# OpenGene/repaq

Hardware: AMD Instinct MI355X
Metric: raw FASTQ MB/s encode+decode (higher is better)
Workload: dtype u8; 1 GPU; configs[2]: synthetic NovaSeq PE150 two files (-i/-I), 2 x 4.01 GB FASTQ (fqgen profile 1, 11200000 pairs, seed 3, N 20 ppm), -k 1000, encode + decode; chunks_per_gpu=3360, parity=unchecked (checked with --full)

## Files before the change

repaq_amd/csrc/enc/gather_tiles.h:

```cpp
#pragma once
#define G2_CAP 23552u
#define G2_SE_OK 1
#define G2_CNT 256u
__device__ __forceinline__ uint32_t ctl_flags4(uint32_t w) { return (w - 0x10101010u) & ~w & 0x80808080u; }
struct __attribute__((packed, aligned(1))) GU16g { uint32_t a, b, c, d; };
__device__ __forceinline__ void pack4_codes(uint32_t w, uint32_t& code, uint32_t& nb, uint32_t& bad) {
    const uint32_t idx = (w >> 1) & 0x03030303u;
    const uint32_t ok = eq_bytes_full(__builtin_amdgcn_perm(0u, 0x47544341u, idx), w);
    code = ((__builtin_amdgcn_perm(0u, 0x00020301u, idx) & ok) * 0x01041040u) >> 24;
    nb = 0; bad = 0;
    if (ok != 0xFFFFFFFFu) { const uint32_t isn = eq_bytes_full(w, 0x4E4E4E4Eu); nb = ((isn & 0x01010101u) * 0x01020408u) >> 24;
            bad = (((~ok & ~isn) & 0x01010101u) * 0x01020408u) >> 24; }
}
__device__ __forceinline__ void pack4_codes_rc(uint32_t w, uint32_t& code, uint32_t& nb) {
    const uint32_t u = w & 0xDFDFDFDFu, idx = (u >> 1) & 0x03030303u;
    const uint32_t ok = eq_bytes_full(__builtin_amdgcn_perm(0u, 0x47544341u, idx), u);
    code = ((__builtin_amdgcn_perm(0u, 0x03010002u, idx) & ok) * 0x01041040u) >> 24;
    nb = ((~ok & 0x01010101u) * 0x01020408u) >> 24;
}
__device__ __forceinline__ bool pack16_fast(const uint32_t (&w)[4], uint32_t& code) {
    uint32_t diff = 0; code = 0;
#pragma unroll
    for (int i = 0; i < 4; i++) {
        const uint32_t idx = (w[i] >> 1) & 0x03030303u;
// ... 461 lines not shown
    G2MRaw mr = g2_mraw(T, pq, gs, j, ntile ? tile_at(1) - gs : 0u);
    if (ntile) g2_stage<SH>(T, two, g2_geo<SH>(b0, b1, two), buf4, tid);
    for (uint32_t t = 0; t < ntile; t++, tix++) {
        const uint32_t cur = tile_at(t), cnt = tile_at(t + 1u) - cur;
        const G2Geo g = g2_geo<SH>(b0, b1, two);
        const G2Read m = g2_read(T, mr, g, f, pq0, il, cur, j, cnt);
        const uint32_t qbeg = b0.q - pq0, qend = b1.q - pq0;
        { const uint32_t ncur = tile_at(t + 1u); mr = g2_mraw(T, pq, ncur, j, tile_at(t + 2u) - ncur); }
        const G2Bound b3 = g2_bound<SH>(T, two, pq, tile_at(t + 3u));
        __syncthreads();
        if (LANES) { if (m.on && (m.gi & 1u)) { const uint32_t ts = m.ssrc + m.len + 1u;
                if (g2_ctl_line(tx, m.nsrc, m.ssrc - 1u - m.nsrc, part, P) | g2_ctl_line(tx, ts, m.qsrc - 1u - ts, part, P)) s_mctl = 1u; } }
        qc.seg0 = qbeg / PC_SEG_POS;
        if (parse && (uint32_t)wave_id() == (tix & 3u)) { g2_parse(T, R, tx, REFN, REFS, g, r0, f, cur, cnt, can0, dpos, dch, acc);
                if (mirror || LANES) g2_mirror_ends(T, tx, g, cur, cnt, M.mirror_err, LANES); }
        if (MASKS) {
            if (tid < nd && s_carry[tid]) atomicOr(&pl[tid * M.pw], s_carry[tid]);
            g2_quals_masks<LANES>(tx, m, part, P, pl, M.pw, qbeg & ~31u, nd, pat0, pat1, pat2, patm, D, qd, gpl, M.pstride, segm + (size_t)c * MAX_STREAMS * n_seg,
                    segc + (size_t)c * MAX_STREAMS * n_seg, n_seg, M.rare + (size_t)c * (1u + G2_RARE_LIST), &s_mctl);
            g2_bases<LANES>(tx, m, part, P, lpk, lnb, rflag, rn, &s_mctl);
        } else g2_compose(tx, m, part, P, qd, lpk, lnb, rflag, rn, qc);
        if (mirror) {
            const uint32_t end1 = g.end1 < T.n[1] ? g.end1 : T.n[1];
            const uint32_t mctl = wave_sum(g2_ctl_count(buf4 + g.base1 / 16u, b0.l1 - g.a01, end1 - g.a01, tid));
            if ((tid & 63u) == 0 && mctl) atomicAdd(&s_mctl, mctl);
            mwant += 2u * cnt - (g.end1 > T.n[1] ? 1u : 0u);
        }
        __syncthreads();
        if (t + 1u < ntile) g2_stage<SH>(T, two, g2_geo<SH>(b1, b2, two), buf4, tid);
        if (MASKS) {
            const uint32_t gw0 = qbeg >> 5, nw = ((qend + 31u) >> 5) - gw0; const bool last_tile = cur + cnt >= ge;
            g2_flush_masks(pl, M.pw, nd, dense3, s_carry, gpl, M.pstride, gw0, nw, !last_tile && (qend & 31u) != 0u, cur == gs && gs > f && (qbeg & 31u) != 0u,
                    last_tile && ge < e && (qend & 31u) != 0u,
                           (size_t)c * MAX_STREAMS * n_seg, n_seg, segm, segc);
        } else qual_flush(sh, sh_last, nrep, nslot, qc.seg0, c, nn_s, segm, segc, n_seg);
        b0 = b1; b1 = b2; b2 = b3;
    }
    if (parse) {
        const uint32_t bits = wave_and(acc.bits), fail = wave_min(acc.fail);
        if ((tid & 63u) == 0) { if (bits != CF_ALL) atomicAnd(&cbits[c], bits); if (fail != 0xFFFFFFFFu) atomicMin(&cfail[c], fail); }
    }
    if (mirror) {
        __syncthreads();
        if (tid == 0 && s_mctl != mwant) atomicOr(M.mirror_err, (uint32_t)DE_MIRROR_FAIL);
    }
    if (LANES) { __syncthreads(); if (tid == 0 && s_mctl) atomicOr(M.mirror_err, (uint32_t)DE_MIRROR_FAIL); }
}
__device__ __forceinline__ uint32_t dense_mask_of(const DevHeader* __restrict__ D, uint32_t nd) { uint32_t m = 0;
        for (uint32_t d = 0; d < nd; d++) m |= 1u << D->dense[d]; return m; }
__device__ __forceinline__ void k_rare_zero_chunk(uint32_t* __restrict__ planes, uint64_t pstride, uint32_t dense_mask, const uint32_t* __restrict__ pq,
        const uint32_t* __restrict__ first, const uint64_t* __restrict__ qbase, uint32_t c) {
    const uint32_t nw = (pq[first[c + 1]] - pq[first[c]] + 31u) >> 5; const size_t w0 = (size_t)(qbase[c] >> 5);
    for (uint32_t v = 0; v < G2_PLANES; v++) if (!((dense_mask >> v) & 1u)) for (uint32_t i = threadIdx.x; i < nw; i += blockDim.x) planes[(size_t)v * pstride + w0 + i] = 0u;
}
__device__ __forceinline__ void nbits_zero_slots(uint16_t* __restrict__ lnb, const uint8_t* __restrict__ rn, const uint32_t* __restrict__ pq, uint32_t g0, uint32_t g1, uint32_t t, uint32_t n) {
    for (uint32_t g = g0 + t; g < g1; g += n) if (rn[g]) { const uint32_t a = pq[g], nw = (pq[g + 1] - a + 15u) >> 4; uint16_t* const o = lnb + (size_t)(a >> 4) + g;
            for (uint32_t i = 0; i < nw; i++) o[i] = 0; }
}
__global__ void k_gather_redo_reset(const uint32_t* __restrict__ only, uint32_t* __restrict__ segm, int* __restrict__ segc, uint32_t n_seg,
                                    uint32_t* __restrict__ xplane, uint64_t pstride, const DevHeader* __restrict__ D, uint32_t nd, const uint32_t* __restrict__ pq, const uint32_t* __restrict__ first, const uint64_t* __restrict__ qbase,
                                    uint16_t* __restrict__ lnb, const uint8_t* __restrict__ rn) {
    const uint32_t c = blockIdx.x; if (!only[c]) return;
    nbits_zero_slots(lnb, rn, pq, first[c], first[c + 1], threadIdx.x, blockDim.x);
    const size_t k = (size_t)c * MAX_STREAMS * n_seg;
    for (uint32_t i = threadIdx.x; i < MAX_STREAMS * n_seg; i += blockDim.x) { segm[k + i] = 0u; segc[k + i] = -1; }
    if (xplane) { k_rare_zero_chunk(xplane, pstride, dense_mask_of(D, nd), pq, first, qbase, c);
            if (threadIdx.x == 0) xplane[(size_t)G2_PLANES * pstride + (size_t)c * (1u + G2_RARE_LIST)] = 0u; }
}
__global__ void k_rare_cleanup(uint32_t* __restrict__ rare, uint32_t* __restrict__ planes, uint64_t pstride, const DevHeader* __restrict__ D, uint32_t nd,
        const uint32_t* __restrict__ pq, const uint32_t* __restrict__ first, const uint64_t* __restrict__ qbase) {
    const uint32_t c = blockIdx.x; uint32_t* const rc = rare + (size_t)c * (1u + G2_RARE_LIST); const uint32_t n = rc[0]; if (!n) return;
    if (n <= G2_RARE_LIST) { const size_t w0 = (size_t)(qbase[c] >> 5); for (uint32_t i = threadIdx.x; i < n; i += blockDim.x) { const uint32_t e = rc[1u + i];
            planes[(size_t)(e >> 28) * pstride + w0 + (e & 0x0FFFFFFFu)] = 0u; } }
    else k_rare_zero_chunk(planes, pstride, dense_mask_of(D, nd), pq, first, qbase, c);
    __syncthreads();
    if (threadIdx.x == 0) rc[0] = 0u;
}
__global__ void __launch_bounds__(256) k_nbits_cleanup(uint16_t* __restrict__ lnb, const uint8_t* __restrict__ rn, const uint32_t* __restrict__ pq, uint32_t n_reads) {
    const uint32_t g0 = 16u * (blockIdx.x * blockDim.x + threadIdx.x); if (g0 >= n_reads) return;
    const uint4 v = *(const uint4*)(rn + g0);
    if (!(v.x | v.y | v.z | v.w)) return;
    nbits_zero_slots(lnb, rn, pq, g0, g0 + 16u < n_reads ? g0 + 16u : n_reads, 0u, 1u);
}
__device__ __forceinline__ uint32_t loose_codes(const uint32_t* __restrict__ lpk, uint32_t ld, uint32_t b) {
    const uint32_t d = ld + (b >> 4), sh = 2u * (b & 15u); const uint32_t lo = lpk[d];
    return sh ? (uint32_t)(((((unsigned long long)lpk[d + 1]) << 32) | lo) >> sh) : lo;
}
__device__ __forceinline__ uint32_t loose_nbits(const uint16_t* __restrict__ lnb, uint32_t ld, uint32_t b) {
    const uint32_t d = ld + (b >> 4), sh = b & 15u; const uint32_t lo = lnb[d];
    return (sh ? ((((uint32_t)lnb[d + 1]) << 16) | lo) >> sh : lo) & 0xFFFFu;
}
#define SP_OWN 4096u
#define SP_EXTRA 8u
#define SP_U 3
struct __attribute__((packed, aligned(4))) SpU8 { uint32_t a, b; };
struct __attribute__((packed, aligned(2))) SpU4 { uint32_t a; };
__global__ void __launch_bounds__(256) k_seqpack(const uint32_t* __restrict__ pq, const uint32_t* __restrict__ sd, const U4* __restrict__ ptot,
        const uint32_t* __restrict__ first, const uint32_t* __restrict__ ilv, const int8_t* __restrict__ ovb,
                                                 const DevHeader* __restrict__ D, const uint64_t* __restrict__ sbase, const uint32_t* __restrict__ lpk, const uint16_t* __restrict__ lnb, const uint8_t* __restrict__ rn,
                                                 uint32_t* __restrict__ spk, uint16_t* __restrict__ snm, uint32_t* __restrict__ ncount, uint32_t* __restrict__ nmap, uint32_t* __restrict__ segm, int* __restrict__ segc, uint32_t n_seg,
                                                 uint32_t rshift) {
    __shared__ uint32_t s_sd[256 + SP_EXTRA + 1], s_ld[256 + SP_EXTRA], s_sk[256 + SP_EXTRA]; __shared__ uint8_t s_own[SP_OWN];
    __shared__ uint8_t s_hn[256 + SP_EXTRA + 8];
    const uint32_t c = blockIdx.y, f = first[c], e = first[c + 1], tid = threadIdx.x;
    const uint32_t ps0 = sd[f], S = ptot[c].d;
    const bool il = ilv[c] != 0, enc = il && (D->flags & H_PE_OVERLAP); const int shift = D->overlap_shift;
    uint32_t* const ok = spk + (size_t)(sbase[c] >> 4); uint16_t* const on = snm + (size_t)(sbase[c] >> 4);
    const uint32_t nshift = nmap_shift(S); uint32_t* const nm = nmap + (size_t)c * NMAP_WORDS;
    const size_t nsi = ((size_t)c * MAX_STREAMS + NPOS_SLOT) * n_seg;
    uint32_t nsum = 0;
    auto skip_of = [&](uint32_t g) -> uint32_t {
        if (enc && ((g - f) & 1u)) { const int ov = (int)ovb[g >> 1] - shift; if (ov > 0) return (uint32_t)ov; }
        return 0u;
    };
    const uint32_t R = 1u << rshift;
    for (uint32_t r0 = f + blockIdx.x * R; r0 < e; r0 += gridDim.x * R) {
        const uint32_t nr = e - r0 < R ? e - r0 : R, nx = e - r0 < R + SP_EXTRA ? e - r0 : R + SP_EXTRA;
        for (uint32_t t = tid; t <= nx; t += blockDim.x) {
            const uint32_t g = r0 + t; s_sd[t] = g < e ? sd[g] - ps0 : S;
            if (t < nx) { s_ld[t] = (pq[g] >> 4) + g; s_sk[t] = skip_of(g); s_hn[t] = rn[g]; } else s_hn[t] = 0;
        }
        __syncthreads();
        const uint32_t kbase = (s_sd[0] + 15u) >> 4, kend = (s_sd[nr] + 15u) >> 4;
        if (tid < nr) { const uint32_t ka = (s_sd[tid] + 15u) >> 4, kb = (s_sd[tid + 1] + 15u) >> 4; for (uint32_t k = ka; k < kb; k++) s_own[k - kbase] = (uint8_t)tid; }
        __syncthreads();
        const uint32_t ndw = kend - kbase;
        for (uint32_t i0 = 0; i0 < ndw; i0 += blockDim.x * SP_U) {
            struct Dw { uint32_t k, need, t1, jj, sh, sh2, take2, n, n2; unsigned long long c, c2; } q[SP_U]; uint32_t nres[SP_U];
#pragma unroll
            for (int u = 0; u < SP_U; u++) nres[u] = 0;
#pragma unroll
            for (int u = 0; u < SP_U; u++) {
                Dw& x = q[u]; x.need = 0; x.take2 = 0; x.k = x.t1 = x.jj = x.sh = x.sh2 = x.n = x.n2 = 0; x.c = x.c2 = 0;
                const uint32_t i = i0 + (uint32_t)u * blockDim.x + tid;
                if (i < ndw) {
                    const uint32_t k = kbase + i, j = s_own[i];
                    const uint32_t B = 16u * k, si = B - s_sd[j], need = S - B < 16u ? S - B : 16u, av = s_sd[j + 1] - B, t1 = need < av ? need : av;
                    const uint32_t b0 = s_sk[j] + si, d = s_ld[j] + (b0 >> 4);
                    x.k = k; x.need = need; x.t1 = t1; x.sh = b0 & 15u; x.jj = j + 1u;
                    { const SpU8 v = *(const SpU8*)(lpk + d); x.c = (((unsigned long long)v.b) << 32) | v.a; x.n = s_hn[j] ? ((const SpU4*)(lnb + d))->a : 0u; }
                    if (t1 < need && j + 1u < nx) {
                        const uint32_t avail = s_sd[j + 2] - s_sd[j + 1]; x.jj = j + 2u;
                        if (avail) {
                            const uint32_t s2 = s_sk[j + 1], d2 = s_ld[j + 1] + (s2 >> 4); x.sh2 = s2 & 15u; x.take2 = avail < need - t1 ? avail : need - t1;
                            const SpU8 v = *(const SpU8*)(lpk + d2); x.c2 = (((unsigned long long)v.b) << 32) | v.a; x.n2 = s_hn[j + 1] ? ((const SpU4*)(lnb + d2))->a : 0u;
                        }
                    }
                }
            }
#pragma unroll
            for (int u = 0; u < SP_U; u++) {
                const Dw& x = q[u];
                if (!x.need) continue;
                const uint32_t k = x.k, B = 16u * k, need = x.need;
                unsigned long long acc = (uint32_t)(x.c >> (2u * x.sh)) & (x.t1 >= 16u ? 0xFFFFFFFFu : (1u << (2u * x.t1)) - 1u);
                uint32_t nacc = ((x.n >> x.sh) & 0xFFFFu) & ((1u << x.t1) - 1u);
                uint32_t filled = x.t1, jj = x.jj;
                if (x.take2) {
                    acc |= (unsigned long long)((uint32_t)(x.c2 >> (2u * x.sh2)) & (x.take2 >= 16u ? 0xFFFFFFFFu : (1u << (2u * x.take2)) - 1u)) << (2u * filled);
                    nacc |= (((x.n2 >> x.sh2) & 0xFFFFu) & ((1u << x.take2) - 1u)) << filled; filled += x.take2;
                }
                while (filled < need) {
                    uint32_t a, b, l2, s2;
                    if (jj < nx) { a = s_sd[jj]; b = s_sd[jj + 1]; l2 = s_ld[jj]; s2 = s_sk[jj]; }
                    else { const uint32_t gg = r0 + jj; a = sd[gg] - ps0; b = gg + 1u < e ? sd[gg + 1] - ps0 : S; l2 = (pq[gg] >> 4) + gg; s2 = skip_of(gg); }
                    const uint32_t avail = b - a;
                    if (avail) {
                        const uint32_t take = avail < need - filled ? avail : need - filled;
                        acc |= (unsigned long long)(loose_codes(lpk, l2, s2) & (take >= 16u ? 0xFFFFFFFFu : (1u << (2u * take)) - 1u)) << (2u * filled);
                        if (jj < nx ? s_hn[jj] : rn[r0 + jj]) nacc |= (loose_nbits(lnb, l2, s2) & ((1u << take) - 1u)) << filled;
                        filled += take;
                    }
                    jj++;
                }
                ok[k] = (uint32_t)acc; on[k] = (uint16_t)nacc; nres[u] = nacc;
            }
#pragma unroll
            for (int u = 0; u < SP_U; u++) {
                const uint32_t na = q[u].need ? nres[u] : 0u;
                const unsigned long long hn = __ballot(na != 0u);
                if (!hn) continue;
                const uint32_t B = 16u * q[u].k, sg = B / PC_SEG_POS, mb = (B >> 12) >> nshift, n = (uint32_t)__popc(na);
                const int lead = __ffsll((long long)hn) - 1;
                const uint32_t sg0 = (uint32_t)__shfl((int)sg, lead), mb0 = (uint32_t)__shfl((int)mb, lead);
                const bool mine = na != 0u && sg == sg0; const int last = na ? (int)(B + 31u - (uint32_t)__clz((int)na)) : -1;
                const uint32_t sum = wave_sum<uint32_t>(mine ? n : 0u); const int mx = wave_max<int>(mine ? last : -1);
                if (lane_id() == lead) { atomicAdd(&segm[nsi + sg0], sum); atomicMax(&segc[nsi + sg0], mx); atomicOr(&nm[mb0 >> 5], 1u << (mb0 & 31u)); }
                if (na != 0u && !mine) { atomicAdd(&segm[nsi + sg], n); atomicMax(&segc[nsi + sg], last); }
                if (na != 0u && mb != mb0) atomicOr(&nm[mb >> 5], 1u << (mb & 31u));
                nsum += n;
            }
        }
        __syncthreads();
    }
    nsum = wave_sum(nsum);
    if (lane_id() == 0 && nsum) atomicAdd(&ncount[c], nsum);
}
__global__ void __launch_bounds__(256) k_packbytes(const U4* __restrict__ pv, const uint32_t* __restrict__ first, const uint64_t* __restrict__ sbase,
        const uint8_t* __restrict__ scat,
                                                   uint32_t* __restrict__ spk, uint16_t* __restrict__ snm) {
    const uint32_t c = blockIdx.y, f = first[c], e = first[c + 1];
    const uint32_t S = pv[e].d - pv[f].d, ndw = (S + 15u) >> 4;
    const uint4* const src = (const uint4*)(scat + sbase[c]);
    uint32_t* const ok = spk + (size_t)(sbase[c] >> 4); uint16_t* const on = snm + (size_t)(sbase[c] >> 4);
    for (uint32_t k = blockIdx.x * blockDim.x + threadIdx.x; k < ndw; k += gridDim.x * blockDim.x) {
        const uint4 v = src[k]; const uint32_t w[4] = { v.x, v.y, v.z, v.w };
        uint32_t code = 0, nbits = 0;
#pragma unroll
        for (int i = 0; i < 4; i++) { uint32_t c4, n4, b4; pack4_codes(w[i], c4, n4, b4); code |= c4 << (8 * i); nbits |= n4 << (4 * i); }
        const uint32_t nv = S - 16u * k;
        if (nv < 16u) { code &= (1u << (2u * nv)) - 1u; nbits &= (1u << nv) - 1u; }
        ok[k] = code; on[k] = (uint16_t)nbits;
    }
}

__global__ void k_stream_plan(ReadTab R, ChunkTab C, const DevHeader* __restrict__ D, uint64_t* __restrict__ ctotal, uint64_t* __restrict__ ctotal_n, uint32_t n_chunks,
        const uint32_t* __restrict__ segm, uint32_t n_seg, int which) {
    const uint32_t c = blockIdx.x; const int l = lane_id();
    if (c >= n_chunks) return;
    const uint32_t f = C.first[c], e = C.first[c + 1];
    const uint32_t len = R.pq[e] - R.pq[f];
    const uint32_t nn = D->n_normal < NPOS_SLOT ? D->n_normal : NPOS_SLOT;
    const bool bycol = (D->flags & H_QUAL_BY_COL) && !(D->flags & H_DONT_QUAL);
    const size_t k = (size_t)c * MAX_STREAMS;
    if (which & 1) {
        auto occ = [&](uint32_t j) -> uint32_t { uint32_t t = 0; const uint32_t* p = segm + ((size_t)c * MAX_STREAMS + j) * n_seg;
                for (uint32_t s_ = 0; s_ < n_seg; s_++) t += p[s_]; return t; };
        const uint32_t ex = bycol ? occ(EXC_SLOT) : 0u;
        const uint32_t pad = PC_SEG_PAD * pc_n_seg(len);
        uint32_t cap = (bycol && (uint32_t)l < nn) ? occ((uint32_t)l) + len / 128 + 3 * (len / 16384) + 16 + pad : 0u;
        const uint32_t al = (cap + 15u) & ~15u;
        const uint32_t incl = wave_incl_sum(al);
        C.scap[k + l] = cap; C.soff[k + l] = incl - al; C.ssize[k + l] = 0;
        const uint32_t run64 = wave_last(incl);
        if (l == 0) { const uint32_t cape = bycol ? 5 * ex + 16 + pad : 0u, ale = (cape + 15u) & ~15u;
                      C.scap[k + EXC_SLOT] = cape; C.soff[k + EXC_SLOT] = run64; C.ssize[k + EXC_SLOT] = 0; ctotal[c] = (uint64_t)run64 + ale; }
    }
    if ((which & 2) && l == 0) {
        const uint32_t slen = C.ptot[c].d, pads = PC_SEG_PAD * pc_n_seg(slen);
        const uint32_t capn = (D->flags & H_N_POS) ? C.ncount[c] + slen / 128 + 3 * (slen / 16384) + 16 + pads : 0u;
        C.scap[k + NPOS_SLOT] = capn; C.soff[k + NPOS_SLOT] = 0; C.ssize[k + NPOS_SLOT] = 0; ctotal_n[c] = (uint64_t)((capn + 15u) & ~15u);
    }
}
```

repaq_amd/csrc/rfq_encode.hip:

```cpp
#include "rfq_ctx.h"
#include <type_traits>
#include "rfq_encode_kernels.h"
#include <algorithm>
#include <cstring>
#include <cstdlib>
#include <cstddef>

enum EncBuf {
    B_BITMAP0 = 0, B_BITMAP1, B_BLK0, B_BLK1, B_LO0, B_LO1, B_SCANTMP,
    B_LEN, B_N1LEN, B_N2OFF, B_X, B_Y, B_TILE, B_LANE, B_OK, B_CHUNK, B_STORED, B_EQ2, B_PQ, B_PV, B_PVIN,
    B_ULEN, B_P, B_MINMAX, B_FIRST, B_CFLAGS, B_IL, B_HIST, B_NCOUNT, B_SCAP, B_SOFF, B_SSIZE, B_XSIZE, B_YSIZE, B_QBASE, B_SBASE,
    B_IMGSIZE, B_IMGOFF, B_CTOTAL, B_CBASE, B_LAYOUT, B_HSTATS, B_OVB, B_OVRAW, B_QCAT, B_SCAT, B_SCRATCH, B_XS, B_YS, B_SEGB, B_SEGC,
    B_NORM0, B_NORM1, B_OT0, B_OT1, B_ONX0, B_ONX1, B_TBITS, B_SBITS, B_NKEEP, B_NTERM, B_NMAP, B_ADJ, B_PINFO, B_SEGM, B_LPK, B_LNB, B_SPK, B_SNM, B_RFLAG, B_SCANTMP2, B_CTOTALN, B_CBASEN, B_SCRATCHN, B_PTOT, B_QPLANE, B_SEGD, B_SEGS, B_SD, B_RN, B_ENC_END
};

static_assert(B_ENC_END <= 80, "encode buffers must stay below the decode buffer indices of rfq_ctx::b");

static int fetch_bytes(rfq_ctx* ctx, const uint8_t* d, size_t n, std::string& out) {
    out.resize(n);
    if (n) HIPCHK(ctx, hipMemcpy(&out[0], d, n, hipMemcpyDeviceToHost));
    return RFQ_OK;
}
static int fetch_line(rfq_ctx* ctx, const Text& T, uint32_t g, int k, std::string& out) {
    int s = 0; uint32_t r = g; if (T.paired == 1) { s = (int)(g & 1u); r = g >> 1; }
// ... 369 lines not shown
}
static int enc_gather_tiles(rfq_ctx* ctx, const EncBatch& b, const EncCut& cut, EncTables& t, EncForm& f, AuxGuard& guard) {
    hipStream_t S = ctx->stream; DBuf* B = ctx->b;
    const uint32_t np = cut.reads_used / 2;
    if (b.mirrored && f.masks && !G2_SE_OK) return RFQ_AGAIN_MIRROR;
    uint8_t *rflag, *rn; HIPCHK(ctx, table(B[B_RFLAG], (t.nr + 15) & ~(size_t)15, rflag)); HIPCHK(ctx, table(B[B_RN], (t.nr + 15) & ~(size_t)15, rn));
    ClearList z; memset(&z, 0, sizeof z);
    if (!(z.add(t.cbits, 2 * t.nc * 4, 0xFFFFFFFFu) && z.add(t.C.ncount, t.nc * 4, 0u) && z.add(t.C.nmap, t.nc * NMAP_WORDS * 4, 0u) && z.add(t.segb, t.nsb * 4, 0u) &&
          z.add(t.segm, t.nsb * 4, 0u) && z.add(t.segc, t.nsb * 4, 0xFFFFFFFFu) && z.add(rflag, t.nr, 0u) && z.add(rn, t.nr, 0u)))
        return rfq_fail(ctx, RFQ_E_HIP, "internal: more than %d regions in one clear list", CLEAR_MAX);
    clear_list(S, z);
    ctx->timer.begin("chunk_flags", S);
    hipLaunchKernelGGL(k_chunk_bases, dim3((cut.n_chunks + 255) / 256), dim3(256), 0, S, t.R, t.C, cut.n_chunks, 1);
    if (f.hdr_aside) HIPCHK(ctx, hipStreamWaitEvent(S, ctx->ev_mid, 0));
    ctx->timer.end(S);

    if (f.masks) { ctx->timer.begin("quality_masks", S); ctx->timer.end(S); }
    ctx->timer.begin("gather", S);
    const size_t nld = (size_t)(cut.total_bases >> 4) + cut.reads_used + 16;
    const size_t lnb_cap = B[B_LNB].cap;
    uint32_t* lpk; uint16_t* lnb; HIPCHK(ctx, table(B[B_LPK], nld * 4, lpk)); HIPCHK(ctx, table(B[B_LNB], nld * 2, lnb));
    if (B[B_LNB].cap != lnb_cap) ctx->lnb_dirty = true;
    if (ctx->lnb_dirty) HIPCHK(ctx, hipMemsetAsync(lnb, 0, B[B_LNB].cap, S));
    ctx->lnb_dirty = true;
    const uint32_t K = 1u << f.kshift;
    const uint32_t bx = grid_x_for(cut.n_chunks, (cut.max_reads + K - 1) / K, 6u * ctx->n_cu);
    const uint32_t text4 = (uint32_t)((((uint64_t)cut.max_rec << f.kshift) + 64u + 15u) / 16u) + 8u;
    G2Planes M; M.planes = nullptr; M.rare = nullptr; M.pstride = 0; M.nd = 0; M.mirror_err = b.mirrored ? &b.dst->err : (uint32_t*)nullptr; M.pw = (uint32_t)((((uint64_t)cut.max_len << f.kshift) + 31u) / 32u) + 2u;
    auto dyn_of = [&](uint32_t nd_) -> uint32_t { return text4 * 16u + (G2_REFN + G2_REFS + 32u) + 4u * nd_ * M.pw; };
    if (f.masks) {
        M.nd = std::min<uint32_t>(ctx->h_hdr.n_normal, 3u);
        if (M.nd == 3u && dyn_of(3u) + 64u > 26880u) M.nd = 2u;
        const size_t need_w = (t.catbytes >> 5) + 16, extra_w = t.nc * (1u + G2_RARE_LIST) / G2_PLANES + 16;
        if (B[B_QPLANE].cap / 4 / G2_PLANES < need_w + extra_w || ctx->qplane_stride < need_w) {
            HIPCHK(ctx, B[B_QPLANE].ensure((need_w + extra_w) * G2_PLANES * 4)); ctx->qplane_stride = B[B_QPLANE].cap / 4 / G2_PLANES - extra_w;
                    ctx->qplane_dirty = true;
        }
        if ((ctx->qplane_stride + extra_w) * G2_PLANES * 4 > B[B_QPLANE].cap) { ctx->qplane_stride = B[B_QPLANE].cap / 4 / G2_PLANES - extra_w;
                ctx->qplane_dirty = true; }
        uint32_t dmask = 0; for (uint32_t d = 0; d < M.nd; d++) dmask |= 1u << (ctx->h_hdr.dense[d] & 7u);
        if (ctx->qplane_mask & ~dmask) ctx->qplane_dirty = true;
        ctx->qplane_mask = dmask;
        M.planes = B[B_QPLANE].as<uint32_t>(); M.pstride = ctx->qplane_stride; M.rare = M.planes + G2_PLANES * M.pstride;
        if (ctx->qplane_dirty) HIPCHK(ctx, hipMemsetAsync(M.planes, 0, ((size_t)M.pstride * G2_PLANES + t.nc * (1u + G2_RARE_LIST)) * 4, S));
        ctx->qplane_dirty = true; ctx->qplane_nd = M.nd;
    }
    t.qplane = f.masks ? M.planes : nullptr;
    const uint32_t dyn = dyn_of(M.nd) + ctx->opt.g2_pad; (void)dyn;
    for (int phase = 1; phase <= (b.is_pe ? 2 : 1); phase++) {
        const uint32_t* only = phase == 2 ? (const uint32_t*)t.redo : (const uint32_t*)nullptr;
        if (phase == 2) hipLaunchKernelGGL(k_gather_redo_reset, dim3(cut.n_chunks), dim3(64), 0, S, only, t.segm, t.segc, t.n_seg,
                                           f.masks ? M.planes : (uint32_t*)nullptr, M.pstride, (const DevHeader*)t.D, M.nd, (const uint32_t*)t.R.pq, (const uint32_t*)t.C.first, (const uint64_t*)t.C.qbase,
                                           lnb, (const uint8_t*)rn);
        if (f.masks) hipLaunchKernelGGL(k_mask_bounds, dim3(cut.n_chunks), dim3(64), 0, S, (const uint32_t*)t.R.pq, (const uint32_t*)t.C.first, (const uint64_t*)t.C.qbase,
                M.planes, M.pstride, (const DevHeader*)t.D, M.nd, bx, only);
#define RFQ_G2_ARGS b.T, t.R, (const uint32_t*)t.C.first, (const uint64_t*)t.C.qbase, (const DevHeader*)t.D, t.qcat, lpk, lnb, rflag, \
                    rn, t.segm, t.segc, t.n_seg, f.kshift, t.cbits, t.cfail, only, text4, M
        if (f.masks && !b.is_pe && G2_SE_OK) hipLaunchKernelGGL((k_gather2<true, 0>), dim3(bx, cut.n_chunks), dim3(256), dyn, S, RFQ_G2_ARGS);
        else if (f.masks && b.a->paired == RFQ_PE_TWO_FILES && G2_SE_OK && b.mirrored) hipLaunchKernelGGL((k_gather2<true, 1, true>), dim3(bx, cut.n_chunks), dim3(256), dyn, S, RFQ_G2_ARGS);
        else if (f.masks && b.a->paired == RFQ_PE_TWO_FILES && G2_SE_OK) hipLaunchKernelGGL((k_gather2<true, 1>), dim3(bx, cut.n_chunks), dim3(256), dyn, S, RFQ_G2_ARGS);
        else if (f.masks) hipLaunchKernelGGL(k_gather2<true>, dim3(bx, cut.n_chunks), dim3(256), dyn, S, RFQ_G2_ARGS);
        else hipLaunchKernelGGL(k_gather2<false>, dim3(bx, cut.n_chunks), dim3(256), dyn, S, RFQ_G2_ARGS);
#undef RFQ_G2_ARGS
        if (phase == 1) hipLaunchKernelGGL(k_chunk_flags_b, dim3(cut.n_chunks), dim3(64), 0, S, t.R, t.C, (const DevHeader*)t.D, b.is_pe ? 1 : 0, (const uint32_t*)t.cbits,
                (const uint32_t*)t.cfail, t.redo);
    }
    HIPCHK(ctx, table(B[B_SCRATCH], std::max<size_t>(B[B_SCRATCH].cap, (size_t)(f.masks ? cut.total_bases / 8 : cut.total_bases + cut.total_bases / 4) + t.nc * 4096 + 256), t.scratch));
    HIPCHK(ctx, table(B[B_SCRATCHN], std::max<size_t>(B[B_SCRATCHN].cap, (size_t)(cut.total_bases / 64) + t.nc * 1024 + 256), t.scratch_n));
    hipLaunchKernelGGL(k_stream_plan, dim3(cut.n_chunks), dim3(64), 0, S, t.R, t.C, (const DevHeader*)t.D, t.ctot, t.ctot_n, cut.n_chunks, (const uint32_t*)t.segm, t.n_seg, 1);
    scan_exclusive<uint64_t>(S, t.ctot, t.cbase, cut.n_chunks, (uint64_t*)t.scantmp, 1);
    hipLaunchKernelGGL(k_enc_totals, dim3(1), dim3(64), 0, S, t.C, (const uint64_t*)t.cbase, cut.n_chunks, 0, b.dst, (uint64_t)B[B_SCRATCH].cap);
    const bool aux_chain = f.aux_chain = ctx->aux_ready() && !ctx->opt.one_stream; hipStream_t A = aux_chain ? ctx->aux : S;
    if (aux_chain) { HIPCHK(ctx, hipEventRecord(ctx->ev_fork, S)); HIPCHK(ctx, hipStreamWaitEvent(A, ctx->ev_fork, 0)); guard.armed = true; }
    if (b.is_pe) {
        const OvLoose Z = { (const uint32_t*)t.R.pq, (const uint32_t*)lpk, (const uint16_t*)lnb, (const uint8_t*)rflag, (const uint8_t*)rn };
        const uint32_t ob = std::min<uint32_t>((np + 255) / 256, 65535u * 16u);
        if (cut.max_len <= 160u) hipLaunchKernelGGL((k_overlap<true, 160u>), dim3(ob), dim3(256), 0, A, b.T, Z, t.ovraw, np);
        else hipLaunchKernelGGL(k_overlap<true>, dim3(ob), dim3(256), 0, A, b.T, Z, t.ovraw, np);
    }
    if (aux_chain) { HIPCHK(ctx, hipEventRecord(ctx->ev_ovl, A)); f.coder_waits = true; }
    hipLaunchKernelGGL(k_chunk_prefix, dim3(cut.n_chunks), dim3(256), 0, A, b.T, t.R, t.C, (const DevHeader*)t.D, (const int16_t*)t.ovraw, t.ovb);
    {
        const uint32_t max_len = cut.max_rec / 2u;
        uint32_t rshift = 8; while (rshift && ((uint64_t)(max_len / 16u + 1u) << rshift) > SP_OWN) rshift--;
        uint32_t sx = grid_x_for(cut.n_chunks, (cut.max_reads >> rshift) + 1u, 8u * ctx->n_cu);
        hipLaunchKernelGGL(k_seqpack, dim3(sx, cut.n_chunks), dim3(256), aux_chain ? ctx->opt.sp_pad : 0u, A, (const uint32_t*)t.R.pq, (const uint32_t*)t.R.sd, (const U4*)t.C.ptot,
                (const uint32_t*)t.C.first, (const uint32_t*)t.C.il, (const int8_t*)t.ovb, (const DevHeader*)t.D,
                           (const uint64_t*)t.C.sbase, (const uint32_t*)lpk, (const uint16_t*)lnb, (const uint8_t*)rn, t.spk, t.snm,
                           t.C.ncount, t.C.nmap, t.segm, t.segc, t.n_seg, rshift);
    }
    uint64_t* tmp2 = B[B_SCANTMP2].as<uint64_t>() + (t.nr / SCAN_TILE + 2) * 2;
    hipLaunchKernelGGL(k_stream_plan, dim3(cut.n_chunks), dim3(64), 0, A, t.R, t.C, (const DevHeader*)t.D, t.ctot, t.ctot_n, cut.n_chunks, (const uint32_t*)t.segm, t.n_seg, 2);
    scan_exclusive<uint64_t>(A, t.ctot_n, t.cbase_n, cut.n_chunks, tmp2, 1);
    chunk_layout(A, b, cut, t, tmp2, 0);
    hipLaunchKernelGGL(k_enc_totals, dim3(1), dim3(64), 0, A, t.C, (const uint64_t*)t.cbase_n, cut.n_chunks, 2, b.dst, (uint64_t)B[B_SCRATCHN].cap);
    KCHK(ctx, "k_gather2");
    ctx->timer.end(S);
    return RFQ_OK;
}
static int enc_gather_bytes(rfq_ctx* ctx, EncBatch& b, const EncCut& cut, EncTables& t, EncForm& f) {
    hipStream_t S = ctx->stream; DBuf* B = ctx->b;
    uint64_t* const tmp = (uint64_t*)t.scantmp;
    HIPCHK(ctx, hipMemsetAsync(t.cbits, 0xFF, 2 * t.nc * 4, S));
    ctx->timer.begin("chunk_flags", S);
    hipLaunchKernelGGL(k_chunk_bases, dim3((cut.n_chunks + 255) / 256), dim3(256), 0, S, t.R, t.C, cut.n_chunks, 1);
    if (f.hdr_aside) HIPCHK(ctx, hipStreamWaitEvent(S, ctx->ev_mid, 0));
    const uint32_t fbx = std::max(1u, std::min<uint32_t>((cut.max_reads + 255) / 256, std::max(1u, 4096u / cut.n_chunks)));
    hipLaunchKernelGGL(k_chunk_flags_a, dim3(fbx, cut.n_chunks), dim3(256), 0, S, b.T, t.R, t.C, (const DevHeader*)t.D, b.is_pe ? 1 : 0, t.cbits, t.cfail);
    hipLaunchKernelGGL(k_chunk_flags_b, dim3(cut.n_chunks), dim3(64), 0, S, t.R, t.C, (const DevHeader*)t.D, b.is_pe ? 1 : 0, (const uint32_t*)t.cbits, (const uint32_t*)t.cfail,
            (uint32_t*)nullptr);
    if (b.is_pe) {
        const OvLoose noz = { nullptr, nullptr, nullptr, nullptr, nullptr };
        const uint32_t ob = std::min<uint32_t>((cut.n_units + 255) / 256, 65535u * 16u);
        hipLaunchKernelGGL(k_overlap<false>, dim3(ob), dim3(256), 0, S, b.T, noz, t.ovraw, cut.n_units);
    }
    const uint32_t np = cut.reads_used / 2; U4* const pvin = B[B_PVIN].as<U4>();
    if (b.is_pe) hipLaunchKernelGGL(k_overlap_apply, dim3((np + 255) / 256), dim3(256), 0, S, t.R, t.C, (const DevHeader*)t.D, (const int16_t*)t.ovraw, t.ovb, np);
    hipLaunchKernelGGL(k_pv_in, dim3((cut.n_reads + 255) / 256), dim3(256), 0, S, b.T, t.R, pvin, cut.n_reads);
    scan_exclusive<U4>(S, pvin, t.R.pv, cut.n_reads, (U4*)t.scantmp, 1);
    hipLaunchKernelGGL(k_chunk_bases, dim3((cut.n_chunks + 255) / 256), dim3(256), 0, S, t.R, t.C, cut.n_chunks, 2);
    hipLaunchKernelGGL(k_chunk_ptot, dim3((cut.n_chunks + 255) / 256), dim3(256), 0, S, t.R, t.C, cut.n_chunks);
    KCHK(ctx, "k_chunk_flags");
    ctx->timer.end(S);

    ctx->timer.begin("gather_bytes", S);
    HIPCHK(ctx, hipMemsetAsync(t.C.ncount, 0, t.nc * 4, S)); HIPCHK(ctx, hipMemsetAsync(t.C.nmap, 0, t.nc * NMAP_WORDS * 4, S));
    HIPCHK(ctx, hipMemsetAsync(t.segb, 0, t.nsb * 4, S)); HIPCHK(ctx, hipMemsetAsync(t.segm, 0, t.nsb * 4, S));
            HIPCHK(ctx, hipMemsetAsync(t.segc, 0xFF, t.nsb * 4, S));
    uint8_t* scat; HIPCHK(ctx, table(B[B_SCAT], t.catbytes, scat));
    const uint32_t bx = grid_x_for(cut.n_chunks, (cut.max_reads + GT_READS - 1) / GT_READS, 5u * ctx->n_cu);
    hipLaunchKernelGGL(k_gather, dim3(bx, cut.n_chunks), dim3(256), 0, S, b.T, t.R, t.C, (const int8_t*)t.ovb, (const DevHeader*)t.D, t.qcat, scat, t.segm, t.segc, t.n_seg);
    const uint32_t px = grid_x_for(cut.n_chunks, (cut.max_chunk_bases / 16u + 255u) / 256u + 1u, 8u * ctx->n_cu);
    hipLaunchKernelGGL(k_packbytes, dim3(px, cut.n_chunks), dim3(256), 0, S, (const U4*)t.R.pv, (const uint32_t*)t.C.first, (const uint64_t*)t.C.sbase, (const uint8_t*)scat,
                       t.spk, t.snm);
    hipLaunchKernelGGL(k_stream_plan, dim3(cut.n_chunks), dim3(64), 0, S, t.R, t.C, (const DevHeader*)t.D, t.ctot, t.ctot_n, cut.n_chunks, (const uint32_t*)t.segm, t.n_seg, 3);
    scan_exclusive<uint64_t>(S, t.ctot, t.cbase, cut.n_chunks, tmp, 1);
    scan_exclusive<uint64_t>(S, t.ctot_n, t.cbase_n, cut.n_chunks, tmp, 1);
    chunk_layout(S, b, cut, t, tmp, 0);
    hipLaunchKernelGGL(k_enc_totals, dim3(1), dim3(64), 0, S, t.C, (const uint64_t*)t.cbase, cut.n_chunks, 0, b.dst, ~0ull);
    hipLaunchKernelGGL(k_enc_totals, dim3(1), dim3(64), 0, S, t.C, (const uint64_t*)t.cbase_n, cut.n_chunks, 2, b.dst, ~0ull);
    KCHK(ctx, "k_gather");
    HIPCHK(ctx, ctx->fetch(&b.hs, b.dst, sizeof b.hs, S));
    if (f.make_header) HIPCHK(ctx, ctx->fetch(&ctx->h_hdr, t.D, sizeof(DevHeader), S));
    HIPCHK(ctx, ctx->fetch_sync(S));
    ctx->timer.end(S);
    { const int rc = header_errors(ctx, b, f); if (rc) return rc; }
    enc_form(ctx, cut, f, true);
    HIPCHK(ctx, table(B[B_SCRATCH], (size_t)b.hs.total_scratch + 256, t.scratch)); HIPCHK(ctx, table(B[B_SCRATCHN], (size_t)b.hs.total_scratch_n + 256, t.scratch_n));
    return RFQ_OK;
}
static int launch_coder(rfq_ctx* ctx, hipStream_t Q, const EncBatch& b, const EncCut& cut, const EncTables& t, const EncForm& f, uint32_t g0, uint32_t gn) {
    if (f.coder_list && g0 == 0 && gn >= f.nqg) {
        const uint64_t mb = (uint64_t)((cut.n_chunks + 7) / 8) * 8ull * t.n_seg;
        if (mb > 0x7FFFFFFFull) return rfq_fail(ctx, RFQ_E_ARG, "batch too large for the position-coder grid");
        hipLaunchKernelGGL(k_pos_coder_list, dim3((uint32_t)mb), dim3(64), std::min<uint32_t>(ctx->h_hdr.n_normal, NPOS_SLOT) * 128u, Q, t.R, t.C, (const DevHeader*)t.D,
                (const uint8_t*)t.qcat, t.scratch, (const uint64_t*)t.cbase, t.segb, (const int*)t.segc, (const uint32_t*)t.segm, t.n_seg, cut.n_chunks, b.dst);
        g0 = f.nqg; gn -= f.nqg;
        if (gn == 0) return RFQ_OK;
    }
    const uint64_t pc_blocks = (uint64_t)((cut.n_chunks + 7) / 8) * 8ull * gn * t.n_seg;
    if (pc_blocks > 0x7FFFFFFFull) return rfq_fail(ctx, RFQ_E_ARG, "batch too large for the position-coder grid");
    hipLaunchKernelGGL(k_pos_coder, dim3((uint32_t)pc_blocks), dim3(64), 0, Q, t.R, t.C, (const DevHeader*)t.D, (const uint8_t*)t.qcat, (const uint16_t*)t.snm,
                       t.scratch, (const uint64_t*)t.cbase, t.scratch_n, (const uint64_t*)t.cbase_n,
                       t.segb, (const int*)t.segc, (const uint32_t*)t.segm, t.n_seg, cut.n_chunks, f.nqg, g0, gn, b.dst,
                       (const uint32_t*)t.qplane, (uint64_t)ctx->qplane_stride);
    return RFQ_OK;
}
// ... 932 lines not shown
```

Before: 1.202 million MB/s.

## Widen seqpack work unit from 16-base dwords to 64-base quads

k_seqpack now has each thread produce a 64-base quad (four packed code dwords plus a 64-bit N mask) instead of one 16-base dword. Each thread loads five code dwords and three N halfwords with wide unaligned loads, then funnel-shifts and masks them branch-free. The goal is fewer threads and iterations per base, wider stores, and fewer per-unit atomics and ballots. The unroll factor drops to 1 and the ownership table shrinks to 1024 entries. The cost is more registers and extra loads past read ends.

Result: no change. 1.199 million MB/s (-0.3%).

```diff
diff --git a/repaq_amd/csrc/enc/gather_tiles.h b/repaq_amd/csrc/enc/gather_tiles.h
--- a/repaq_amd/csrc/enc/gather_tiles.h
+++ b/repaq_amd/csrc/enc/gather_tiles.h
@@ -567,19 +567,21 @@
     if (!(v.x | v.y | v.z | v.w)) return;
     nbits_zero_slots(lnb, rn, pq, g0, g0 + 16u < n_reads ? g0 + 16u : n_reads, 0u, 1u);
 }
-__device__ __forceinline__ uint32_t loose_codes(const uint32_t* __restrict__ lpk, uint32_t ld, uint32_t b) {
-    const uint32_t d = ld + (b >> 4), sh = 2u * (b & 15u); const uint32_t lo = lpk[d];
-    return sh ? (uint32_t)(((((unsigned long long)lpk[d + 1]) << 32) | lo) >> sh) : lo;
-}
-__device__ __forceinline__ uint32_t loose_nbits(const uint16_t* __restrict__ lnb, uint32_t ld, uint32_t b) {
-    const uint32_t d = ld + (b >> 4), sh = b & 15u; const uint32_t lo = lnb[d];
-    return (sh ? ((((uint32_t)lnb[d + 1]) << 16) | lo) >> sh : lo) & 0xFFFFu;
-}
-#define SP_OWN 4096u
+#define SP_OWN 1024u
 #define SP_EXTRA 8u
-#define SP_U 3
-struct __attribute__((packed, aligned(4))) SpU8 { uint32_t a, b; };
-struct __attribute__((packed, aligned(2))) SpU4 { uint32_t a; };
+#define SP_U 1
+static_assert(PC_SEG_POS % 64u == 0u && 4096u % 64u == 0u, "a quad lies in one coder segment and under one bit of the N map");
+struct __attribute__((packed, aligned(4))) SpU20 { uint32_t a, b, c, d, e; };
+struct __attribute__((packed, aligned(2))) SpN12 { uint32_t a, b, c; };
+struct Sp5 { uint32_t a, c, e, b, d; }; struct Sp3 { uint32_t a, b, c; };
+__device__ __forceinline__ Sp5 sp_load(const uint32_t* __restrict__ p) { const SpU20* const v = (const SpU20*)p; Sp5 r; r.a = v->a; r.b = v->b; r.c = v->c; r.d = v->d; r.e = v->e; return r; }
+__device__ __forceinline__ Sp3 sp_load(const uint16_t* __restrict__ p) { const SpN12* const v = (const SpN12*)p; return Sp3{ v->a, v->b, v->c }; }
+__device__ __forceinline__ uint32_t sp_funnel(uint32_t lo, uint32_t hi, uint32_t sh) { return (uint32_t)(((((unsigned long long)hi) << 32) | lo) >> (2u * (sh & 15u))); }
+__device__ __forceinline__ void sp_codes(const Sp5& v, uint32_t sh, uint32_t (&o)[4]) { o[0] = sp_funnel(v.a, v.b, sh); o[1] = sp_funnel(v.b, v.c, sh); o[2] = sp_funnel(v.c, v.d, sh); o[3] = sp_funnel(v.d, v.e, sh); }
+__device__ __forceinline__ unsigned long long sp_nbits(const Sp3& v, uint32_t sh) {
+    return (((((unsigned long long)v.b) << 32) | v.a) >> sh) | ((((unsigned long long)v.c) << 1) << (63u - sh)); }
+__device__ __forceinline__ uint32_t sp_below(uint32_t t, uint32_t i) { return t <= 16u * i ? 0u : t >= 16u * i + 16u ? 0xFFFFFFFFu : (1u << (2u * (t - 16u * i))) - 1u; }
+__device__ __forceinline__ unsigned long long sp_below64(uint32_t t) { return t >= 64u ? ~0ull : (1ull << t) - 1ull; }
 __global__ void __launch_bounds__(256) k_seqpack(const uint32_t* __restrict__ pq, const uint32_t* __restrict__ sd, const U4* __restrict__ ptot,
         const uint32_t* __restrict__ first, const uint32_t* __restrict__ ilv, const int8_t* __restrict__ ovb,
                                                  const DevHeader* __restrict__ D, const uint64_t* __restrict__ sbase, const uint32_t* __restrict__ lpk, const uint16_t* __restrict__ lnb, const uint8_t* __restrict__ rn,
@@ -606,73 +608,70 @@
             if (t < nx) { s_ld[t] = (pq[g] >> 4) + g; s_sk[t] = skip_of(g); s_hn[t] = rn[g]; } else s_hn[t] = 0;
         }
         __syncthreads();
-        const uint32_t kbase = (s_sd[0] + 15u) >> 4, kend = (s_sd[nr] + 15u) >> 4;
-        if (tid < nr) { const uint32_t ka = (s_sd[tid] + 15u) >> 4, kb = (s_sd[tid + 1] + 15u) >> 4; for (uint32_t k = ka; k < kb; k++) s_own[k - kbase] = (uint8_t)tid; }
+        const uint32_t kbase = (s_sd[0] + 63u) >> 6, kend = (s_sd[nr] + 63u) >> 6;
+        if (tid < nr) { const uint32_t ka = (s_sd[tid] + 63u) >> 6, kb = (s_sd[tid + 1] + 63u) >> 6; for (uint32_t k = ka; k < kb; k++) s_own[k - kbase] = (uint8_t)tid; }
         __syncthreads();
-        const uint32_t ndw = kend - kbase;
-        for (uint32_t i0 = 0; i0 < ndw; i0 += blockDim.x * SP_U) {
-            struct Dw { uint32_t k, need, t1, jj, sh, sh2, take2, n, n2; unsigned long long c, c2; } q[SP_U]; uint32_t nres[SP_U];
-#pragma unroll
-            for (int u = 0; u < SP_U; u++) nres[u] = 0;
+        const uint32_t nq = kend - kbase;
+        for (uint32_t i0 = 0; i0 < nq; i0 += blockDim.x * SP_U) {
+            struct Qd { uint32_t k, need, t1, filled, jj, sh, sh2; Sp5 c, c2; Sp3 n, n2; } q[SP_U]; unsigned long long nres[SP_U];
 #pragma unroll
             for (int u = 0; u < SP_U; u++) {
-                Dw& x = q[u]; x.need = 0; x.take2 = 0; x.k = x.t1 = x.jj = x.sh = x.sh2 = x.n = x.n2 = 0; x.c = x.c2 = 0;
+                Qd& x = q[u]; x = Qd{}; nres[u] = 0;
                 const uint32_t i = i0 + (uint32_t)u * blockDim.x + tid;
-                if (i < ndw) {
+                if (i < nq) {
                     const uint32_t k = kbase + i, j = s_own[i];
-                    const uint32_t B = 16u * k, si = B - s_sd[j], need = S - B < 16u ? S - B : 16u, av = s_sd[j + 1] - B, t1 = need < av ? need : av;
-                    const uint32_t b0 = s_sk[j] + si, d = s_ld[j] + (b0 >> 4);
-                    x.k = k; x.need = need; x.t1 = t1; x.sh = b0 & 15u; x.jj = j + 1u;
-                    { const SpU8 v = *(const SpU8*)(lpk + d); x.c = (((unsigned long long)v.b) << 32) | v.a; x.n = s_hn[j] ? ((const SpU4*)(lnb + d))->a : 0u; }
+                    const uint32_t B = 64u * k, need = S - B < 64u ? S - B : 64u, av = s_sd[j + 1] - B, t1 = need < av ? need : av;
+                    const uint32_t b0 = s_sk[j] + (B - s_sd[j]), d = s_ld[j] + (b0 >> 4);
+                    x.k = k; x.need = need; x.t1 = x.filled = t1; x.sh = b0 & 15u; x.jj = j + 1u;
+                    x.c = sp_load(lpk + d); if (s_hn[j]) x.n = sp_load(lnb + d);
                     if (t1 < need && j + 1u < nx) {
                         const uint32_t avail = s_sd[j + 2] - s_sd[j + 1]; x.jj = j + 2u;
                         if (avail) {
-                            const uint32_t s2 = s_sk[j + 1], d2 = s_ld[j + 1] + (s2 >> 4); x.sh2 = s2 & 15u; x.take2 = avail < need - t1 ? avail : need - t1;
-                            const SpU8 v = *(const SpU8*)(lpk + d2); x.c2 = (((unsigned long long)v.b) << 32) | v.a; x.n2 = s_hn[j + 1] ? ((const SpU4*)(lnb + d2))->a : 0u;
+                            const uint32_t e2 = s_sk[j + 1] + 64u - t1, d2 = s_ld[j + 1] + (e2 >> 4) - 4u; x.sh2 = e2 & 15u; x.filled = t1 + (avail < need - t1 ? avail : need - t1);
+                            x.c2 = sp_load(lpk + d2); if (s_hn[j + 1]) x.n2 = sp_load(lnb + d2);
                         }
                     }
                 }
             }
 #pragma unroll
             for (int u = 0; u < SP_U; u++) {
-                const Dw& x = q[u];
+                const Qd& x = q[u];
                 if (!x.need) continue;
-                const uint32_t k = x.k, B = 16u * k, need = x.need;
-                unsigned long long acc = (uint32_t)(x.c >> (2u * x.sh)) & (x.t1 >= 16u ? 0xFFFFFFFFu : (1u << (2u * x.t1)) - 1u);
-                uint32_t nacc = ((x.n >> x.sh) & 0xFFFFu) & ((1u << x.t1) - 1u);
-                uint32_t filled = x.t1, jj = x.jj;
-                if (x.take2) {
-                    acc |= (unsigned long long)((uint32_t)(x.c2 >> (2u * x.sh2)) & (x.take2 >= 16u ? 0xFFFFFFFFu : (1u << (2u * x.take2)) - 1u)) << (2u * filled);
-                    nacc |= (((x.n2 >> x.sh2) & 0xFFFFu) & ((1u << x.take2) - 1u)) << filled; filled += x.take2;
-                }
+                const uint32_t need = x.need;
+                uint32_t acc[4], o2[4], filled = x.filled, jj = x.jj; sp_codes(x.c, x.sh, acc); sp_codes(x.c2, x.sh2, o2);
+#pragma unroll
+                for (int i = 0; i < 4; i++) { const uint32_t m1 = sp_below(x.t1, i); acc[i] = ((acc[i] & m1) | (o2[i] & ~m1)) & sp_below(filled, i); }
+                unsigned long long nacc; { const unsigned long long m1 = sp_below64(x.t1); nacc = ((sp_nbits(x.n, x.sh) & m1) | (sp_nbits(x.n2, x.sh2) & ~m1)) & sp_below64(filled); }
                 while (filled < need) {
                     uint32_t a, b, l2, s2;
                     if (jj < nx) { a = s_sd[jj]; b = s_sd[jj + 1]; l2 = s_ld[jj]; s2 = s_sk[jj]; }
                     else { const uint32_t gg = r0 + jj; a = sd[gg] - ps0; b = gg + 1u < e ? sd[gg + 1] - ps0 : S; l2 = (pq[gg] >> 4) + gg; s2 = skip_of(gg); }
                     const uint32_t avail = b - a;
                     if (avail) {
-                        const uint32_t take = avail < need - filled ? avail : need - filled;
-                        acc |= (unsigned long long)(loose_codes(lpk, l2, s2) & (take >= 16u ? 0xFFFFFFFFu : (1u << (2u * take)) - 1u)) << (2u * filled);
-                        if (jj < nx ? s_hn[jj] : rn[r0 + jj]) nacc |= (loose_nbits(lnb, l2, s2) & ((1u << take) - 1u)) << filled;
-                        filled += take;
+                        const uint32_t to = filled + (avail < need - filled ? avail : need - filled), e2 = s2 + 64u - filled, d2 = l2 + (e2 >> 4) - 4u;
+                        sp_codes(sp_load(lpk + d2), e2 & 15u, o2); Sp3 vn = Sp3{}; if (jj < nx ? s_hn[jj] : rn[r0 + jj]) vn = sp_load(lnb + d2);
+#pragma unroll
+                        for (int i = 0; i < 4; i++) acc[i] |= o2[i] & ~sp_below(filled, i) & sp_below(to, i);
+                        nacc |= sp_nbits(vn, e2 & 15u) & ~sp_below64(filled) & sp_below64(to);
+                        filled = to;
                     }
                     jj++;
                 }
-                ok[k] = (uint32_t)acc; on[k] = (uint16_t)nacc; nres[u] = nacc;
+                *(uint4*)(ok + 4u * (size_t)x.k) = make_uint4(acc[0], acc[1], acc[2], acc[3]); *(unsigned long long*)(on + 4u * (size_t)x.k) = nacc; nres[u] = nacc;
             }
 #pragma unroll
             for (int u = 0; u < SP_U; u++) {
-                const uint32_t na = q[u].need ? nres[u] : 0u;
-                const unsigned long long hn = __ballot(na != 0u);
+                const unsigned long long na = q[u].need ? nres[u] : 0ull;
+                const unsigned long long hn = __ballot(na != 0ull);
                 if (!hn) continue;
-                const uint32_t B = 16u * q[u].k, sg = B / PC_SEG_POS, mb = (B >> 12) >> nshift, n = (uint32_t)__popc(na);
+                const uint32_t B = 64u * q[u].k, sg = B / PC_SEG_POS, mb = (B >> 12) >> nshift, n = (uint32_t)__popcll(na);
                 const int lead = __ffsll((long long)hn) - 1;
                 const uint32_t sg0 = (uint32_t)__shfl((int)sg, lead), mb0 = (uint32_t)__shfl((int)mb, lead);
-                const bool mine = na != 0u && sg == sg0; const int last = na ? (int)(B + 31u - (uint32_t)__clz((int)na)) : -1;
+                const bool mine = na != 0ull && sg == sg0; const int last = na ? (int)(B + 63u - (uint32_t)__clzll((long long)na)) : -1;
                 const uint32_t sum = wave_sum<uint32_t>(mine ? n : 0u); const int mx = wave_max<int>(mine ? last : -1);
                 if (lane_id() == lead) { atomicAdd(&segm[nsi + sg0], sum); atomicMax(&segc[nsi + sg0], mx); atomicOr(&nm[mb0 >> 5], 1u << (mb0 & 31u)); }
-                if (na != 0u && !mine) { atomicAdd(&segm[nsi + sg], n); atomicMax(&segc[nsi + sg], last); }
-                if (na != 0u && mb != mb0) atomicOr(&nm[mb >> 5], 1u << (mb & 31u));
+                if (na != 0ull && !mine) { atomicAdd(&segm[nsi + sg], n); atomicMax(&segc[nsi + sg], last); }
+                if (na != 0ull && mb != mb0) atomicOr(&nm[mb >> 5], 1u << (mb & 31u));
                 nsum += n;
             }
         }
diff --git a/repaq_amd/csrc/rfq_encode.hip b/repaq_amd/csrc/rfq_encode.hip
--- a/repaq_amd/csrc/rfq_encode.hip
+++ b/repaq_amd/csrc/rfq_encode.hip
@@ -475,7 +475,7 @@
     hipLaunchKernelGGL(k_chunk_prefix, dim3(cut.n_chunks), dim3(256), 0, A, b.T, t.R, t.C, (const DevHeader*)t.D, (const int16_t*)t.ovraw, t.ovb);
     {
         const uint32_t max_len = cut.max_rec / 2u;
-        uint32_t rshift = 8; while (rshift && ((uint64_t)(max_len / 16u + 1u) << rshift) > SP_OWN) rshift--;
+        uint32_t rshift = 8; while (rshift && ((uint64_t)(max_len / 64u + 1u) << rshift) > SP_OWN) rshift--;
         uint32_t sx = grid_x_for(cut.n_chunks, (cut.max_reads >> rshift) + 1u, 8u * ctx->n_cu);
         hipLaunchKernelGGL(k_seqpack, dim3(sx, cut.n_chunks), dim3(256), aux_chain ? ctx->opt.sp_pad : 0u, A, (const uint32_t*)t.R.pq, (const uint32_t*)t.R.sd, (const U4*)t.C.ptot,
                 (const uint32_t*)t.C.first, (const uint32_t*)t.C.il, (const int8_t*)t.ovb, (const DevHeader*)t.D,
```
